# wangty537/raft_optical_flow

Hardware: AMD Instinct MI355X
Metric: image-pairs/s at Sintel 436x1024, 32 iters; corr-lookup GB/s vs HBM peak (higher is better)
Workload: dtype fp32 (convs: f16x3 split MFMA, fp32 accumulate); 1 GPU; RAFT-full inference, 436x1024 padded to 440x1024, 1 pair(s)/GPU/step, iters=32, all-pairs corr, hipGraph; global_batch=1, parallelism=frame-pair sharding x1

## Files before the change

raft_optical_flow_amd/csrc/lookup_conv.hip:

```cpp
#include "lookup_common.hpp"

namespace raft {
namespace {

constexpr int LC_TH = 2, LC_TW = 16, LC_M = 32;
constexpr int LC_R = 4, LC_L = 4, LC_RD = 9;
constexpr int LC_NTAP = LC_L * LC_RD * LC_RD;
constexpr int LC_KS = (LC_NTAP + 31) / 32;
constexpr int LC_N = 256;
constexpr int LC_F1N = 128;
constexpr int LC_F1K = 7, LC_F1KK = 49;
constexpr int LC_F1KS = (2 * LC_F1KK + 31) / 32;
constexpr int LC_FPH = LC_TH + LC_F1K - 1, LC_FPW = LC_TW + LC_F1K - 1;
constexpr int LC_PX = 4;

constexpr int LC_A_BYTES = LC_KS * LC_M * 128;
constexpr int LC_A1_BYTES = LC_F1KS * LC_M * 128;
constexpr int LC_FL_BYTES = LC_FPH * LC_FPW * 8;
constexpr int LC_PATCH_FLOATS = 16 * patch_rs<4>();
constexpr int LC_PATCH_BYTES = 8 * 2 * LC_PATCH_FLOATS * 4;
constexpr int LC_YT_BYTES = 8 * LC_PX * LC_L * LC_RD * 16;
constexpr int LC_OFF_A1 = LC_A_BYTES, LC_OFF_FL = LC_OFF_A1 + LC_A1_BYTES, LC_OFF_PATCH = LC_OFF_FL + LC_FL_BYTES,
              LC_OFF_YT = LC_OFF_PATCH + LC_PATCH_BYTES, LC_LDS = LC_OFF_YT + LC_YT_BYTES;
static_assert(LC_LDS <= 160 * 1024, "LDS budget");

struct LookupConvArgs {
  LookupArgs a;
  const h8* wfrag;
  const float* bias;
  float* out;
  int out_ld;
  int* out_flag;
  const h8* f1frag;
  const float* f1bias;
  float* f1out;
  int f1out_ld;
  int* f1flag;
  int tx_n, ty_n;
  int span_slot;
};

constexpr int LC_SPAN_SLOTS = 256;
__device__ unsigned long long g_lc_span[2 * LC_SPAN_SLOTS];
int g_lc_span_next = -1;

__device__ __forceinline__ void wave_sync() {
  __builtin_amdgcn_fence(__ATOMIC_RELEASE, "wavefront");
  __builtin_amdgcn_wave_barrier();
  __builtin_amdgcn_fence(__ATOMIC_ACQUIRE, "wavefront");
}

template <bool X3, bool BF>
__device__ __forceinline__ void split1(float x, _Float16& hi, _Float16& lo) {
  if constexpr (BF) {
    hi = __builtin_bit_cast(_Float16, (__bf16)x);
  } else {
    hi = (_Float16)x;
    if constexpr (X3) lo = (_Float16)(x - (float)hi);
  }
}

#ifdef LC_STAMPS
__device__ unsigned long long g_lcstamp[16 * 16384];
__device__ __forceinline__ unsigned long long lc_clock() {
  unsigned long long t;
  __builtin_amdgcn_sched_barrier(0);
  asm volatile("s_memtime %0\n\ts_waitcnt lgkmcnt(0)" : "=s"(t)::"memory");
  __builtin_amdgcn_sched_barrier(0);
  return t;
}
__device__ __forceinline__ unsigned long long lc_real() {
  unsigned long long t;
  __builtin_amdgcn_sched_barrier(0);
  asm volatile("s_memrealtime %0\n\ts_waitcnt lgkmcnt(0)" : "=s"(t)::"memory");
  __builtin_amdgcn_sched_barrier(0);
  return t;
}
#define LC_STAMP(k) lc_t[k] = lc_clock()
#else
#define LC_STAMP(k)
#endif

template <int PREC>
__global__ __launch_bounds__(512) void lookup_conv_kernel(LookupConvArgs g) {
#ifdef LC_STAMPS
  unsigned long long lc_t[10];
  const unsigned long long lc_r0 = lc_real();
  LC_STAMP(0);
#endif
  constexpr bool X3 = PREC == RAFT_PREC_F16X3;
  constexpr bool BF = PREC == RAFT_PREC_BF16;
  constexpr int NT = X3 ? 4 : 2;
  constexpr int R = LC_R, RD = LC_RD, WD = 2 * R + 2, RS = patch_rs<4>();
  __shared__ __attribute__((aligned(1024))) char smem[LC_LDS];
  const LookupArgs& a = g.a;
  const int lane = threadIdx.x & 63;
  const int wv = __builtin_amdgcn_readfirstlane(threadIdx.x >> 6);
  const int tile = xcd_tile(blockIdx.x, gridDim.x);
  if (g.span_slot >= 0 && threadIdx.x == 0)
    atomicMin(&g_lc_span[2 * g.span_slot], (unsigned long long)__builtin_amdgcn_s_memrealtime());
  const int per = g.tx_n * g.ty_n;
  const int b = tile / per, sr = tile - b * per;
  const int y0 = (sr / g.tx_n) * LC_TH, x0 = (sr % g.tx_n) * LC_TW;
  const int H = a.H, W = a.W, P = H * W;

#ifndef LC_PF
#define LC_PF 3
#endif
#ifndef LC_TAPS2
#define LC_TAPS2 1
#endif
#ifndef LC_A1EARLY
#define LC_A1EARLY 0
#endif
  constexpr int PF = LC_PF;
  h8 wb[PF + 1][NT];
  auto load_w = [&](int j, h8 (&dst)[NT]) {
    const h8* wf = j < LC_KS ? g.wfrag + ((j * (LC_N / 32) + wv) * 4) * 64
                             : g.f1frag + (((j - LC_KS) * (LC_F1N / 32) + wv) * 4) * 64;
#pragma unroll
    for (int t = 0; t < NT; ++t) dst[t] = wf[t * 64 + lane];
  };

  const int ti = lane >> 4, tj = (lane >> 2) & 3, rr = lane & 3;
  const int lrow = ti * 4 + rr;
  int lth[LC_L], ltw[LC_L];
  unsigned lmsz[LC_L];
  const float* lbs[LC_L];
#pragma unroll
  for (int l = 0; l < LC_L; ++l) {
    lth[l] = a.lv[l].th;
    ltw[l] = a.lv[l].tw;
    lmsz[l] = (unsigned)a.lv[l].mapsz;
    lbs[l] = a.lbase[l];
  }
  float px_x[LC_PX], px_y[LC_PX];
  int px_gp[LC_PX];
  bool px_ok[LC_PX];
#pragma unroll
  for (int k = 0; k < LC_PX; ++k) {
    const int mk = LC_PX * wv + k;
    const int yy = y0 + (mk >> 4), xx = x0 + (mk & 15);
    const bool ok = yy < H && xx < W;
    px_ok[k] = ok;
    px_gp[k] = ok ? b * P + yy * W + xx : b * P;
  }
  {
    int gk = px_gp[0];
#pragma unroll
    for (int k = 1; k < LC_PX; ++k) gk = (lane & 3) == k ? px_gp[k] : gk;
    const float cx = a.coords[2L * gk], cy = a.coords[2L * gk + 1];
#ifdef LC_EARLY
    __builtin_amdgcn_sched_barrier(0);
#pragma unroll
    for (int j = 0; j < PF; ++j) load_w(j, wb[j]);
    __builtin_amdgcn_sched_barrier(0);
#endif
#pragma unroll
    for (int k = 0; k < LC_PX; ++k) {
      px_x[k] = __int_as_float(__builtin_amdgcn_readlane(__float_as_int(cx), k));
      px_y[k] = __int_as_float(__builtin_amdgcn_readlane(__float_as_int(cy), k));
    }
  }
#ifdef LC_STAMPS
  asm volatile("" ::"v"(px_x[0]), "v"(px_y[LC_PX - 1]));
  LC_STAMP(7);
#endif
  const bool col = lane < LC_L * RD;
  int lq = 0;
#pragma unroll
  for (int k = 1; k < LC_L; ++k) lq += lane >= k * RD ? 1 : 0;
  const int l = col ? lq : 0;
  const int ix = lane - l * RD;
  const f32x4 prm = a.prm[l];
  const int fi = threadIdx.x;
  const int fyy = y0 - 3 + fi / LC_FPW, fxx = x0 - 3 + fi % LC_FPW;
  const bool fin = fi < LC_FPH * LC_FPW && (unsigned)fyy < (unsigned)H && (unsigned)fxx < (unsigned)W;
  f32x2 fc = {0.f, 0.f};
  if (fin) fc = *reinterpret_cast<const f32x2*>(a.coords + 2L * ((long)b * P + fyy * W + fxx));
  const int m = lane & 31, h = lane >> 5;
  const float c1b = g.bias ? g.bias[32 * wv + m] : 0.f;
  const float f1b = (wv < 4 && g.f1bias) ? g.f1bias[32 * wv + m] : 0.f;
#ifndef LC_EARLYWAIT
#define LC_EARLYWAIT 1
#endif
  if constexpr (LC_EARLYWAIT != 0) asm volatile("" ::"v"(prm), "v"(c1b), "v"(f1b), "v"(fc));

  __builtin_amdgcn_sched_barrier(0);
  f32x4 v[LC_PX][LC_L];
#ifndef LC_OFF32
#define LC_OFF32 1
#endif
#ifndef LC_TAB
#define LC_TAB 1
#endif
  bool off32 = LC_OFF32 != 0;
  const unsigned nmaps = (unsigned)(a.B * P);
#pragma unroll
  for (int l = 0; l < LC_L; ++l) off32 &= (unsigned long long)nmaps * lmsz[l] * 4ull < 0x7FFFFFF0ull;
  if (off32) {
    __amdgpu_buffer_rsrc_t rsl[LC_L];
    unsigned lano[LC_L], lmsz4[LC_L];
#pragma unroll
    for (int l = 0; l < LC_L; ++l) {
      rsl[l] = __builtin_amdgcn_make_buffer_rsrc(const_cast<float*>(lbs[l]), (short)0, (int)(nmaps * lmsz[l] * 4u),
                                                 0x00020000);
      lano[l] = __umul24((unsigned)ti, (unsigned)(64 * ltw[l])) + 16u * (unsigned)(lane & 15);
      lmsz4[l] = lmsz[l] * 4u;
    }
#if LC_TAB
    int t_sb, t_row, t_col;
    {
      const int ik = (lane >> 2) & 3, il = lane & 3;
      float fx = px_x[0], fy = px_y[0];
      int gpk = px_gp[0];
      bool okk = px_ok[0];
#pragma unroll
      for (int k = 1; k < LC_PX; ++k) {
        fx = ik == k ? px_x[k] : fx;
        fy = ik == k ? px_y[k] : fy;
        gpk = ik == k ? px_gp[k] : gpk;
        okk = ik == k ? px_ok[k] : okk;
      }
      int thl = lth[0], twl = ltw[0];
      unsigned msl = lmsz4[0];
#pragma unroll
      for (int l = 1; l < LC_L; ++l) {
        thl = il == l ? lth[l] : thl;
        twl = il == l ? ltw[l] : twl;
        msl = il == l ? lmsz4[l] : msl;
      }
      const int wx0 = (floor_origin(fx) >> il) - R, wy0 = (floor_origin(fy) >> il) - R;
      const int tyo = wy0 >> 2, txo = wx0 >> 2;
      const int ntx = ((wx0 + WD - 1) >> 2) - txo + 1;
      const int rlo = max(wy0, 0), rhi = min(wy0 + WD, 4 * thl);
      const int clo = max(txo, 0), chi = min(txo + ntx, twl);
      const int rn = okk ? max(rhi - rlo, 0) : 0, cn = max(chi - clo, 0);
      t_sb = (int)((unsigned)gpk * msl + (unsigned)(tyo * twl + txo) * 64u);
      t_row = ((rlo - 4 * tyo) & 0xFFFF) | (rn << 16);
      t_col = ((clo - txo) & 0xFFFF) | (cn << 16);
    }
#pragma unroll
    for (int k = 0; k < LC_PX; ++k) {
#pragma unroll
      for (int l = 0; l < LC_L; ++l) {
        const unsigned sb = (unsigned)__builtin_amdgcn_readlane(t_sb, 4 * k + l);
        const int rp = __builtin_amdgcn_readlane(t_row, 4 * k + l), cp = __builtin_amdgcn_readlane(t_col, 4 * k + l);
        const bool tok = ((unsigned)(lrow - (rp & 0xFFFF)) < (unsigned)(rp >> 16)) &
                         ((unsigned)(tj - (cp & 0xFFFF)) < (unsigned)(cp >> 16));
        unsigned offv = sb + lano[l];
        asm volatile("" : "+v"(offv));
        const unsigned off = tok ? offv : 0x80000000u;
        v[k][l] = __builtin_bit_cast(f32x4, __builtin_amdgcn_raw_buffer_load_b128(rsl[l], off, 0, 0));
      }
    }
#else
#pragma unroll
    for (int k = 0; k < LC_PX; ++k) {
      const unsigned gp = (unsigned)px_gp[k];
      const int xf = __builtin_amdgcn_readfirstlane(floor_origin(px_x[k]));
      const int yf = __builtin_amdgcn_readfirstlane(floor_origin(px_y[k]));
#pragma unroll
      for (int l = 0; l < LC_L; ++l) {
        const int wx0 = (xf >> l) - R, wy0 = (yf >> l) - R;
        const int tyo = wy0 >> 2, txo = wx0 >> 2;
        const int ntx = ((wx0 + WD - 1) >> 2) - txo + 1;
        const int rowm = 4 * tyo + lrow, colt = txo + tj;
        const bool tok = px_ok[k] & ((unsigned)(rowm - wy0) < (unsigned)WD) & ((unsigned)rowm < (unsigned)(4 * lth[l])) &
                         ((unsigned)tj < (unsigned)ntx) & ((unsigned)colt < (unsigned)ltw[l]);
        const unsigned sb = gp * lmsz4[l] + (unsigned)(tyo * ltw[l] + txo) * 64u;
        unsigned offv = sb + lano[l];
        asm volatile("" : "+v"(offv));
        const unsigned off = tok ? offv : 0x80000000u;
        v[k][l] = __builtin_bit_cast(f32x4, __builtin_amdgcn_raw_buffer_load_b128(rsl[l], off, 0, 0));
      }
    }
#endif
  } else {
#if LC_TAB
    int t_lo, t_hi, t_row, t_col;
    {
      const int ik = (lane >> 2) & 3, il = lane & 3;
      float fx = px_x[0], fy = px_y[0];
      int gpk = px_gp[0];
      bool okk = px_ok[0];
#pragma unroll
      for (int k = 1; k < LC_PX; ++k) {
        fx = ik == k ? px_x[k] : fx;
        fy = ik == k ? px_y[k] : fy;
        gpk = ik == k ? px_gp[k] : gpk;
        okk = ik == k ? px_ok[k] : okk;
      }
      int thl = lth[0], twl = ltw[0];
      unsigned msl = lmsz[0];
      const float* bsl = lbs[0];
#pragma unroll
      for (int l = 1; l < LC_L; ++l) {
        thl = il == l ? lth[l] : thl;
        twl = il == l ? ltw[l] : twl;
        msl = il == l ? lmsz[l] : msl;
        bsl = il == l ? lbs[l] : bsl;
      }
      const int wx0 = (floor_origin(fx) >> il) - R, wy0 = (floor_origin(fy) >> il) - R;
      const int tyo = wy0 >> 2, txo = wx0 >> 2;
      const int ntx = ((wx0 + WD - 1) >> 2) - txo + 1;
      const int rlo = max(wy0, 0), rhi = min(wy0 + WD, 4 * thl);
      const int clo = max(txo, 0), chi = min(txo + ntx, twl);
      const int rn = okk ? max(rhi - rlo, 0) : 0, cn = max(chi - clo, 0);
      const float* wbase = bsl + (long)((unsigned long long)(unsigned)gpk * msl) + ((long)tyo * twl + txo) * 16;
      const unsigned long long wa = reinterpret_cast<unsigned long long>(wbase);
      t_lo = (int)(unsigned)wa;
      t_hi = (int)(unsigned)(wa >> 32);
      t_row = ((rlo - 4 * tyo) & 0xFFFF) | (rn << 16);
      t_col = ((clo - txo) & 0xFFFF) | (cn << 16);
    }
#pragma unroll
    for (int k = 0; k < LC_PX; ++k) {
#pragma unroll
      for (int l = 0; l < LC_L; ++l) {
        const unsigned lo = (unsigned)__builtin_amdgcn_readlane(t_lo, 4 * k + l);
        const unsigned hi = (unsigned)__builtin_amdgcn_readlane(t_hi, 4 * k + l);
        const int rp = __builtin_amdgcn_readlane(t_row, 4 * k + l), cp = __builtin_amdgcn_readlane(t_col, 4 * k + l);
        const bool tok = ((unsigned)(lrow - (rp & 0xFFFF)) < (unsigned)(rp >> 16)) &
                         ((unsigned)(tj - (cp & 0xFFFF)) < (unsigned)(cp >> 16));
        const float* wbase = reinterpret_cast<const float*>(((unsigned long long)hi << 32) | lo);
        const __amdgpu_buffer_rsrc_t rs =
            __builtin_amdgcn_make_buffer_rsrc(const_cast<float*>(wbase), (short)0, 0x7FFFFFFF, 0x00020000);
        unsigned offv = __umul24((unsigned)ti, (unsigned)(64 * ltw[l])) + 16u * (unsigned)(lane & 15);
        asm volatile("" : "+v"(offv));
        const unsigned off = tok ? offv : 0x80000000u;
        v[k][l] = __builtin_bit_cast(f32x4, __builtin_amdgcn_raw_buffer_load_b128(rs, off, 0, 0));
      }
    }
#else
#pragma unroll
  for (int k = 0; k < LC_PX; ++k) {
    const bool ok = px_ok[k];
    const int gp = px_gp[k];
    const int xf = __builtin_amdgcn_readfirstlane(floor_origin(px_x[k]));
    const int yf = __builtin_amdgcn_readfirstlane(floor_origin(px_y[k]));
#pragma unroll
    for (int l = 0; l < LC_L; ++l) {
      const int wx0 = (xf >> l) - R, wy0 = (yf >> l) - R;
      const int tyo = wy0 >> 2, txo = wx0 >> 2;
      const int ntx = ((wx0 + WD - 1) >> 2) - txo + 1;
      const int rlo = max(wy0, 0), rhi = min(wy0 + WD, 4 * lth[l]);
      const int clo = max(txo, 0), chi = min(txo + ntx, ltw[l]);
      const int rb = __builtin_amdgcn_readfirstlane(rlo - 4 * tyo), cb = __builtin_amdgcn_readfirstlane(clo - txo);
      const bool tok = ok && ((unsigned)(lrow - rb) < (unsigned)max(rhi - rlo, 0)) &&
                       ((unsigned)(tj - cb) < (unsigned)max(chi - clo, 0));
      const float* wbase = lbs[l] + (long)((unsigned long long)(unsigned)gp * lmsz[l]) + ((long)tyo * ltw[l] + txo) * 16;
      const __amdgpu_buffer_rsrc_t rs =
          __builtin_amdgcn_make_buffer_rsrc(const_cast<float*>(wbase), (short)0, 0x7FFFFFFF, 0x00020000);
      const unsigned off = tok ? __umul24((unsigned)ti, (unsigned)(64 * ltw[l])) + 16u * (unsigned)(lane & 15)
                               : 0x80000000u;
      v[k][l] = __builtin_bit_cast(f32x4, __builtin_amdgcn_raw_buffer_load_b128(rs, off, 0, 0));
    }
  }
#endif
  }
  LC_STAMP(1);
  int4* ytab = reinterpret_cast<int4*>(smem + LC_OFF_YT) + wv * LC_PX * LC_L * RD;
  int xw[LC_PX], xi[LC_PX];
  float xt[LC_PX];
  bool onp[LC_PX];
#pragma unroll
  for (int k = 0; k < LC_PX; ++k) {
    const float s = __builtin_ldexpf(1.0f, -l);
    const int xf = __builtin_amdgcn_readfirstlane(floor_origin(px_x[k]));
    const int yf = __builtin_amdgcn_readfirstlane(floor_origin(px_y[k]));
    axis_entry<R>(px_x[k] * s, xf >> l, ix, prm[0], prm[1], xw[k], xt[k], xi[k]);
    int yw, yi;
    float yt;
    axis_entry<R, true>(px_y[k] * s, yf >> l, ix, prm[2], prm[3], yw, yt, yi);
    onp[k] = xw[k] >= 0 && yw >= 0;
    if (col) ytab[k * LC_L * RD + lane] = int4{yw >= 0 ? yw * RS * 4 : yw, __float_as_int(yt), __float_as_int(1.0f - yt), yi};
  }
  float2* fl = reinterpret_cast<float2*>(smem + LC_OFF_FL);
  if (fi < LC_FPH * LC_FPW) {
    float2 fv = {0.f, 0.f};
    if (fin) {
      fv.x = fc[0] - (float)fxx;
      fv.y = fc[1] - (float)fyy;
    }
    fl[fi] = fv;
  }
  LC_STAMP(2);
#if LC_A1EARLY
  __syncthreads();
  {
    const int mm = threadIdx.x >> 4, q = threadIdx.x & 15;
    const int py = mm >> 4, px = mm & 15;
    float e[8];
#pragma unroll
    for (int i = 0; i < 8; ++i) {
      const int k = 8 * q + i, t = k >> 1;
      const int dy = t / LC_F1K, dx = t - dy * LC_F1K;
      const float2 fv = fl[(py + (k < 2 * LC_F1KK ? dy : 0)) * LC_FPW + px + (k < 2 * LC_F1KK ? dx : 0)];
      e[i] = k < 2 * LC_F1KK ? ((k & 1) ? fv.y : fv.x) : 0.f;
    }
    h8 hi, lo;
    split8<X3, BF>(f32x4{e[0], e[1], e[2], e[3]}, f32x4{e[4], e[5], e[6], e[7]}, hi, lo);
    const int j = q >> 2, qd = q & 3, sw = (mm >> 1) & 7;
    char* row = smem + LC_OFF_A1 + j * (LC_M * 128) + mm * 128;
    *reinterpret_cast<h8*>(row + ((qd ^ sw) << 4)) = hi;
    if constexpr (X3) *reinterpret_cast<h8*>(row + (((4 + qd) ^ sw) << 4)) = lo;
  }
#endif

#ifndef LC_EARLY
#pragma unroll
  for (int j = 0; j < PF; ++j) load_w(j, wb[j]);
#endif
  char* Abase = smem;
  bool big = false;
  auto patch_of = [&](int k) {
    return reinterpret_cast<float*>(smem + LC_OFF_PATCH) + (wv * 2 + (k & 1)) * LC_PATCH_FLOATS;
  };
  const int cbase = l * RD * RD + ix * RD;
  auto taps = [&](int k, float (&val)[RD]) {
    const float* patch = patch_of(k);
    const int4* yt = ytab + k * LC_L * RD;
    const float ex = 1.0f - xt[k];
    const int xwk = xw[k];
    if (__all(!col || onp[k])) {
      if (col) {
        const char* p0 = reinterpret_cast<const char*>(&patch[pidx<4>(0, xwk, l)]);
        const char* p1 = reinterpret_cast<const char*>(&patch[pidx<4>(0, xwk + 1, l)]);
        auto at = [](const char* bp, int byte) { return *reinterpret_cast<const float*>(bp + byte); };
#ifndef LC_TAPS3
#define LC_TAPS3 1
#endif
#if LC_TAPS3 && LC_TAPS2
        int ro[RD];
        float tyv[RD];
        bool cons = true;
#pragma unroll
        for (int iy = 0; iy < RD; ++iy) {
          const int2 ye = *reinterpret_cast<const int2*>(&yt[l * RD + iy]);
          ro[iy] = ye.x;
          tyv[iy] = __int_as_float(ye.y);
        }
#pragma unroll
        for (int iy = 1; iy < RD; ++iy) cons &= ro[iy] == ro[0] + iy * (4 * RS);
        if (__all(cons)) {
          const char* q0 = p0 + ro[0];
          const char* q1 = p1 + ro[0];
          float a0[RD + 1], a1[RD + 1];
#pragma unroll
          for (int r = 0; r <= RD; ++r) {
            a0[r] = at(q0, r * (4 * RS));
            a1[r] = at(q1, r * (4 * RS));
          }
#pragma unroll
          for (int iy = 0; iy < RD; ++iy) {
            const float ty = tyv[iy], sS = 1.0f - ty;
            const f32x2 c0 = {a0[iy], a0[iy + 1]}, c1 = {a1[iy], a1[iy + 1]};
            const f32x2 hh = __builtin_elementwise_fma(c0, (f32x2){ex, ex}, c1 * (f32x2){xt[k], xt[k]});
            val[iy] = fmaf(sS, hh.x, ty * hh.y);
          }
        } else {
#pragma unroll
          for (int iy = 0; iy < RD; ++iy) {
            const float ty = tyv[iy], sS = 1.0f - ty;
            const f32x2 c0 = {at(p0, ro[iy]), at(p0, ro[iy] + 4 * RS)}, c1 = {at(p1, ro[iy]), at(p1, ro[iy] + 4 * RS)};
            const f32x2 hh = __builtin_elementwise_fma(c0, (f32x2){ex, ex}, c1 * (f32x2){xt[k], xt[k]});
            val[iy] = fmaf(sS, hh.x, ty * hh.y);
          }
        }
#else
#pragma unroll
        for (int iy = 0; iy < RD; ++iy) {
#if LC_TAPS2
          const int2 ye = *reinterpret_cast<const int2*>(&yt[l * RD + iy]);
          const int ro = ye.x;
          const float ty = __int_as_float(ye.y), sS = 1.0f - ty;
#else
          const int4 ye = yt[l * RD + iy];
          const int ro = ye.x;
          const float ty = __int_as_float(ye.y), sS = __int_as_float(ye.z);
#endif
          const f32x2 c0 = {at(p0, ro), at(p0, ro + 4 * RS)}, c1 = {at(p1, ro), at(p1, ro + 4 * RS)};
          const f32x2 hh = __builtin_elementwise_fma(c0, (f32x2){ex, ex}, c1 * (f32x2){xt[k], xt[k]});
          val[iy] = fmaf(sS, hh.x, ty * hh.y);
        }
#ifndef LC_TAPSGB
#define LC_TAPSGB 1
#endif
#if LC_TAPSGB && LC_TAPS2
        __builtin_amdgcn_sched_group_barrier(0x100, RD, 0);
        __builtin_amdgcn_sched_group_barrier(0x100, 2 * RD, 0);
        __builtin_amdgcn_sched_group_barrier(0x002, 4 * RD, 0);
#endif
#endif
      }
    } else if (col) {
      unsigned deferred = 0;
#pragma unroll
      for (int iy = 0; iy < RD; ++iy) {
        const int4 ye = yt[l * RD + iy];
        const int yw2 = ye.x;
        const float ty = __int_as_float(ye.y), sS = __int_as_float(ye.z);
        const bool on = (xwk | yw2) >= 0;
        const bool nan = xwk == NAN_POS || yw2 == NAN_POS;
        const int r0 = on ? yw2 / (4 * RS) : 0, c0 = on ? xwk : 0;
        const float vv = patch[pidx<4>(r0, c0, l)] * (sS * ex) + patch[pidx<4>(r0, c0 + 1, l)] * (sS * xt[k]) +
                         patch[pidx<4>(r0 + 1, c0, l)] * (ty * ex) + patch[pidx<4>(r0 + 1, c0 + 1, l)] * (ty * xt[k]);
        val[iy] = nan ? __builtin_nanf("") : vv;
        deferred |= (!on && !nan) ? 1u << iy : 0u;
      }
      if (deferred != 0) {
        const Level& lvl = a.lv[l];
        const float* mp = a.pyr + lvl.off + (long)px_gp[k] * lvl.mapsz;
        auto at = [&](int yy, int xx) {
          return ((unsigned)yy < (unsigned)lvl.h && (unsigned)xx < (unsigned)lvl.w) ? mp[tiled_index(yy, xx, lvl.tw)]
                                                                                    : 0.f;
        };
#pragma unroll
        for (int iy = 0; iy < RD; ++iy) {
          if (!((deferred >> iy) & 1u)) continue;
          const int4 ye = yt[l * RD + iy];
          const int yi = ye.w;
          const float ty = __int_as_float(ye.y), sS = __int_as_float(ye.z);
          val[iy] = at(yi, xi[k]) * (sS * ex) + at(yi, xi[k] + 1) * (sS * xt[k]) + at(yi + 1, xi[k]) * (ty * ex) +
                    at(yi + 1, xi[k] + 1) * (ty * xt[k]);
        }
      }
    }
  };
  auto write_row = [&](int k, const float (&val)[RD]) {
    const int mk = LC_PX * wv + k;
    const int sw = (mk >> 1) & 7;
#if LC_TAPS2
    if (col) {
      const int par = cbase & 1;
      float vv[RD];
#pragma unroll
      for (int iy = 0; iy < RD; ++iy) {
        vv[iy] = px_ok[k] ? val[iy] : 0.f;
        big |= fabsf(vv[iy]) > RAFT_RANGE_LIMIT;
      }
      auto at_c = [&](int c, int half) {
        const int j = c >> 5, kk = c & 31;
        return Abase + j * (LC_M * 128) + mk * 128 + (((4 * half + (kk >> 3)) ^ sw) << 4) + 2 * (kk & 7);
      };
#pragma unroll
      for (int q = 0; q < 4; ++q) {
        const float a0 = par ? vv[2 * q + 1] : vv[2 * q], a1 = par ? vv[2 * q + 2] : vv[2 * q + 1];
        _Float16 h0, l0, h1, l1;
        split1<X3, BF>(a0, h0, l0);
        split1<X3, BF>(a1, h1, l1);
        const int c = cbase + 2 * q + par;
        *reinterpret_cast<h2*>(at_c(c, 0)) = h2{h0, h1};
        if constexpr (X3) *reinterpret_cast<h2*>(at_c(c, 1)) = h2{l0, l1};
      }
      {
        const float a = par ? vv[0] : vv[RD - 1];
        _Float16 hs, ls;
        split1<X3, BF>(a, hs, ls);
        const int c = cbase + (par ? 0 : RD - 1);
        *reinterpret_cast<_Float16*>(at_c(c, 0)) = hs;
        if constexpr (X3) *reinterpret_cast<_Float16*>(at_c(c, 1)) = ls;
      }
    } else if (lane - LC_L * RD < 32 * LC_KS - LC_NTAP) {
#else
    if (col) {
#pragma unroll
      for (int iy = 0; iy < RD; ++iy) {
        const float vv = px_ok[k] ? val[iy] : 0.f;
        big |= fabsf(vv) > RAFT_RANGE_LIMIT;
        const int c = cbase + iy;
        const int j = c >> 5, kk = c & 31;
        _Float16 hi, lo;
        split1<X3, BF>(vv, hi, lo);
        char* rb = Abase + j * (LC_M * 128) + mk * 128;
        *reinterpret_cast<_Float16*>(rb + (((kk >> 3) ^ sw) << 4) + 2 * (kk & 7)) = hi;
        if constexpr (X3) *reinterpret_cast<_Float16*>(rb + (((4 + (kk >> 3)) ^ sw) << 4) + 2 * (kk & 7)) = lo;
      }
    } else if (lane - LC_L * RD < 32 * LC_KS - LC_NTAP) {
#endif
      const int c = LC_NTAP + lane - LC_L * RD;
      const int j = c >> 5, kk = c & 31;
      char* rb = Abase + j * (LC_M * 128) + mk * 128;
      *reinterpret_cast<_Float16*>(rb + (((kk >> 3) ^ sw) << 4) + 2 * (kk & 7)) = (_Float16)0.f;
      if constexpr (X3) *reinterpret_cast<_Float16*>(rb + (((4 + (kk >> 3)) ^ sw) << 4) + 2 * (kk & 7)) = (_Float16)0.f;
    }
    if (a.flow && lane < 2 && px_ok[k]) {
      const int p = px_gp[k] - b * P;
      const float gcoord = lane == 0 ? (float)(p % W) : (float)(p / W);
      a.flow[(long)px_gp[k] * a.flow_ld + lane] = (lane == 0 ? px_x[k] : px_y[k]) - gcoord;
    }
  };
#pragma unroll
  for (int k = 0; k < LC_PX; k += 2) {
#pragma unroll
    for (int lv_ = 0; lv_ < LC_L; ++lv_) {
      *reinterpret_cast<f32x4*>(&patch_of(k)[pidx<4>(lrow, tj * 4, lv_)]) = v[k][lv_];
      *reinterpret_cast<f32x4*>(&patch_of(k + 1)[pidx<4>(lrow, tj * 4, lv_)]) = v[k + 1][lv_];
    }
    wave_sync();
    float va[RD], vb[RD];
    taps(k, va);
    taps(k + 1, vb);
    write_row(k, va);
    write_row(k + 1, vb);
    wave_sync();
  }
  if (a.range_flag && big) *a.range_flag = 1;
  LC_STAMP(3);
#if LC_A1EARLY
  __syncthreads();
#else
  __syncthreads();
  {
    const int mm = threadIdx.x >> 4, q = threadIdx.x & 15;
    const int py = mm >> 4, px = mm & 15;
    float e[8];
#pragma unroll
    for (int i = 0; i < 8; ++i) {
      const int k = 8 * q + i, t = k >> 1;
      const int dy = t / LC_F1K, dx = t - dy * LC_F1K;
      const float2 fv = fl[(py + (k < 2 * LC_F1KK ? dy : 0)) * LC_FPW + px + (k < 2 * LC_F1KK ? dx : 0)];
      e[i] = k < 2 * LC_F1KK ? ((k & 1) ? fv.y : fv.x) : 0.f;
    }
    h8 hi, lo;
    split8<X3, BF>(f32x4{e[0], e[1], e[2], e[3]}, f32x4{e[4], e[5], e[6], e[7]}, hi, lo);
    const int j = q >> 2, qd = q & 3, sw = (mm >> 1) & 7;
    char* row = smem + LC_OFF_A1 + j * (LC_M * 128) + mm * 128;
    *reinterpret_cast<h8*>(row + ((qd ^ sw) << 4)) = hi;
    if constexpr (X3) *reinterpret_cast<h8*>(row + (((4 + qd) ^ sw) << 4)) = lo;
  }
  __syncthreads();
#endif
  LC_STAMP(4);

  const int sw = (m >> 1) & 7;
  auto kstep = [&](const char* A, const h8 (&B)[NT], f32x16& c, f32x16& cx) {
    const char* row = A + m * 128;
    h8 ah[2], al[2];
#pragma unroll
    for (int qq = 0; qq < 2; ++qq) {
      ah[qq] = *reinterpret_cast<const h8*>(row + (((2 * h + qq) ^ sw) << 4));
      if constexpr (X3) al[qq] = *reinterpret_cast<const h8*>(row + (((4 + 2 * h + qq) ^ sw) << 4));
    }
#pragma unroll
    for (int qq = 0; qq < 2; ++qq) {
      if constexpr (BF) {
        c = __builtin_amdgcn_mfma_f32_32x32x16_bf16(__builtin_bit_cast(bf8, ah[qq]), __builtin_bit_cast(bf8, B[qq]), c,
                                                    0, 0, 0);
      } else {
        c = __builtin_amdgcn_mfma_f32_32x32x16_f16(ah[qq], B[qq], c, 0, 0, 0);
      }
      if constexpr (X3) {
        cx = __builtin_amdgcn_mfma_f32_32x32x16_f16(ah[qq], B[2 + qq], cx, 0, 0, 0);
        c = __builtin_amdgcn_mfma_f32_32x32x16_f16(al[qq], B[qq], c, 0, 0, 0);
      }
    }
  };
  f32x16 acc = {}, accx = {}, facc = {}, faccx = {};
  const bool f1w = wv < LC_F1N / 32;
#ifndef LC_SGB
#define LC_SGB 1
#endif
  if constexpr (LC_SGB) {
    struct AF {
      h8 ah[2], al[2];
    };
    auto read_af = [&](const char* A, AF& f) {
      const char* row = A + m * 128;
#pragma unroll
      for (int qq = 0; qq < 2; ++qq) {
        f.ah[qq] = *reinterpret_cast<const h8*>(row + (((2 * h + qq) ^ sw) << 4));
        if constexpr (X3) f.al[qq] = *reinterpret_cast<const h8*>(row + (((4 + 2 * h + qq) ^ sw) << 4));
      }
    };
    auto mfma_af = [&](const AF& f, const h8 (&B)[NT], f32x16& c, f32x16& cx) {
#pragma unroll
      for (int qq = 0; qq < 2; ++qq) {
        if constexpr (BF) {
          c = __builtin_amdgcn_mfma_f32_32x32x16_bf16(__builtin_bit_cast(bf8, f.ah[qq]), __builtin_bit_cast(bf8, B[qq]),
                                                      c, 0, 0, 0);
        } else {
          c = __builtin_amdgcn_mfma_f32_32x32x16_f16(f.ah[qq], B[qq], c, 0, 0, 0);
        }
        if constexpr (X3) {
          cx = __builtin_amdgcn_mfma_f32_32x32x16_f16(f.ah[qq], B[2 + qq], cx, 0, 0, 0);
          c = __builtin_amdgcn_mfma_f32_32x32x16_f16(f.al[qq], B[qq], c, 0, 0, 0);
        }
      }
    };
    auto load_w_any = [&](int j, h8 (&dst)[NT]) {
      const int wq = j < LC_KS ? wv : (wv < LC_F1N / 32 ? wv : LC_F1N / 32 - 1);
      const h8* wf = j < LC_KS ? g.wfrag + ((j * (LC_N / 32) + wq) * 4) * 64
                               : g.f1frag + (((j - LC_KS) * (LC_F1N / 32) + wq) * 4) * 64;
#pragma unroll
      for (int t = 0; t < NT; ++t) dst[t] = wf[t * 64 + lane];
    };
    constexpr int NRA = X3 ? 4 : 2, NMA = X3 ? 6 : 2;
    auto groups = [&](bool loads) {
      if (loads) __builtin_amdgcn_sched_group_barrier(0x020, NT, 0);
#pragma unroll
      for (int i = 0; i < NMA; ++i) {
        if (i < NRA) __builtin_amdgcn_sched_group_barrier(0x100, 1, 0);
        __builtin_amdgcn_sched_group_barrier(0x008, 1, 0);
      }
    };
    AF af[2];
    read_af(Abase, af[0]);
#pragma unroll
    for (int j = 0; j < LC_KS; ++j) {
      __builtin_amdgcn_sched_barrier(0);
      if (j + PF < LC_KS + LC_F1KS) load_w_any(j + PF, wb[(j + PF) % (PF + 1)]);
      read_af(j + 1 < LC_KS ? Abase + (j + 1) * (LC_M * 128) : smem + LC_OFF_A1, af[(j + 1) & 1]);
      mfma_af(af[j & 1], wb[j % (PF + 1)], acc, accx);
      groups(j + PF < LC_KS + LC_F1KS);
      __builtin_amdgcn_sched_barrier(0);
    }
    if (f1w) {
#pragma unroll
      for (int j = LC_KS; j < LC_KS + LC_F1KS; ++j) {
        __builtin_amdgcn_sched_barrier(0);
        if (j + PF < LC_KS + LC_F1KS) load_w_any(j + PF, wb[(j + PF) % (PF + 1)]);
        if (j + 1 < LC_KS + LC_F1KS) read_af(smem + LC_OFF_A1 + (j + 1 - LC_KS) * (LC_M * 128), af[(j + 1) & 1]);
        mfma_af(af[j & 1], wb[j % (PF + 1)], facc, faccx);
        __builtin_amdgcn_sched_barrier(0);
      }
    }
  } else {
#pragma unroll
  for (int j = 0; j < LC_KS; ++j) {
    if (j + PF < LC_KS || f1w) load_w(j + PF, wb[(j + PF) % (PF + 1)]);
    kstep(Abase + j * (LC_M * 128), wb[j % (PF + 1)], acc, accx);
  }
  if (f1w) {
#pragma unroll
    for (int j = LC_KS; j < LC_KS + LC_F1KS; ++j) {
      if (j + PF < LC_KS + LC_F1KS) load_w(j + PF, wb[(j + PF) % (PF + 1)]);
      kstep(smem + LC_OFF_A1 + (j - LC_KS) * (LC_M * 128), wb[j % (PF + 1)], facc, faccx);
    }
  }
  }
  if constexpr (X3) {
#pragma unroll
    for (int r = 0; r < 16; ++r) {
      acc[r] += accx[r] * (1.0f / SPLIT_SCALE);
      facc[r] += faccx[r] * (1.0f / SPLIT_SCALE);
    }
  }
#ifdef LC_STAMPS
  asm volatile("" ::"v"(acc[0]), "v"(acc[15]), "v"(facc[0]));
#endif
  LC_STAMP(5);

  auto store = [&](const f32x16& c, float bias, float* out, int ld, int n, int* flag) {
    bool obig = false;
#pragma unroll
    for (int r = 0; r < 16; ++r) {
      const int mm = (r & 3) + 8 * (r >> 2) + 4 * h;
      const int yy = y0 + (mm >> 4), xx = x0 + (mm & 15);
      const float o = fmaxf(c[r] + bias, 0.f);
      if (yy < H && xx < W) {
        obig |= o > RAFT_RANGE_LIMIT;
        out[((long)b * P + yy * W + xx) * ld + n] = o;
      }
    }
    if (flag && obig) *flag = 1;
  };
  store(acc, c1b, g.out, g.out_ld, 32 * wv + m, g.out_flag);
  if (wv < LC_F1N / 32) store(facc, f1b, g.f1out, g.f1out_ld, 32 * wv + m, g.f1flag);
  if (g.span_slot >= 0) {
    __builtin_amdgcn_s_waitcnt(0);
    __syncthreads();
    if (threadIdx.x == 0)
      atomicMax(&g_lc_span[2 * g.span_slot + 1], (unsigned long long)__builtin_amdgcn_s_memrealtime());
  }
#ifdef LC_END_FENCE
  __builtin_amdgcn_fence(__ATOMIC_RELEASE, "agent");
  __builtin_amdgcn_s_waitcnt(0);
#endif
#ifdef LC_STAMPS
  __builtin_amdgcn_s_waitcnt(0);
  LC_STAMP(6);
  const unsigned long long lc_r1 = lc_real();
  const unsigned wid = blockIdx.x * 8 + wv;
  if (lane == 0 && wid < 16384) {
    unsigned long long* gs = g_lcstamp + wid * 16;
    gs[0] = lc_r0;
    gs[1] = lc_r1;
    for (int k = 0; k < 7; ++k) gs[2 + k] = lc_t[k];
    gs[9] = lc_t[7];
  }
#endif
}

__global__ void lookup_conv_pack_kernel(const h8* __restrict__ split, int k_steps, int nsub, h8* __restrict__ out) {
  const int i = blockIdx.x * blockDim.x + threadIdx.x;
  const int total = k_steps * nsub * 4 * 64;
  if (i >= total) return;
  const int lane = i & 63, t = (i >> 6) & 3, rest = i >> 8;
  const int s = rest % nsub, j = rest / nsub;
  const int n = 32 * s + (lane & 31), hh = lane >> 5, qq = t & 1, lo = t >> 1;
  out[i] = split[((long)n * k_steps + j) * 8 + lo * 4 + 2 * hh + qq];
}

}
}

using namespace raft;

#ifdef LC_STAMPS
extern "C" int raft_debug_lcstamps(unsigned long long* host, int n) {
  return (int)hipMemcpyFromSymbol(host, HIP_SYMBOL(g_lcstamp), sizeof(unsigned long long) * (size_t)n);
}
#endif

extern "C" size_t raft_lookup_conv_weight_floats(int n, int k_pad) {
  if (n <= 0 || n % 32 || k_pad <= 0) return 0;
  return (size_t)((k_pad + 31) / 32) * (size_t)n * 32;
}

extern "C" int raft_lookup_conv_pack_weight(const void* split_weight, int n_pad, int k_pad, int n, void* out,
                                            raft_stream_t stream) {
  RAFT_REQUIRE(split_weight && out && n > 0 && n % 32 == 0 && n <= n_pad && k_pad > 0 && k_pad % 32 == 0,
               "raft_lookup_conv_pack_weight: bad arguments");
  RAFT_REQUIRE((((uintptr_t)split_weight | (uintptr_t)out) & 15) == 0, "raft_lookup_conv_pack_weight: 16-B alignment");
  const int ks = k_pad / 32, nsub = n / 32;
  const int total = ks * nsub * 256;
  hipLaunchKernelGGL(lookup_conv_pack_kernel, dim3((unsigned)cdiv(total, 256)), dim3(256), 0, as_stream(stream),
                     reinterpret_cast<const h8*>(split_weight), ks, nsub, reinterpret_cast<h8*>(out));
  return check_launch("raft_lookup_conv_pack_weight");
}

extern "C" int raft_corr_lookup_conv(const float* pyramid, int B, int H, int W, int L, int radius, const float* coords,
                                     float* flow_out, int flow_ld, int* range_flag, int precision,
                                     const void* c1_weight, const float* c1_bias, int c1_n, float* c1_out,
                                     int c1_out_ld, int* c1_range_flag, const void* f1_weight, const float* f1_bias,
                                     int f1_n, int f1_k, float* f1_out, int f1_out_ld, int* f1_range_flag,
                                     raft_stream_t stream) {
  RAFT_REQUIRE(L == LC_L && radius == LC_R, "raft_corr_lookup_conv: radius 4 and 4 levels only (got %d, %d)", radius,
               L);
  RAFT_REQUIRE(c1_n == LC_N && f1_n == LC_F1N && f1_k == LC_F1K,
               "raft_corr_lookup_conv: convc1 256 / convf1 128 outputs, convf1 7x7 only");
  RAFT_REQUIRE(precision == RAFT_PREC_F16X3 || precision == RAFT_PREC_F16 || precision == RAFT_PREC_BF16,
               "raft_corr_lookup_conv: precision must be F16X3, F16 or BF16 (got %d)", precision);
  RAFT_REQUIRE(c1_weight && c1_out && c1_out_ld >= c1_n && f1_weight && f1_out && f1_out_ld >= f1_n,
               "raft_corr_lookup_conv: bad conv arguments");
  RAFT_REQUIRE((((uintptr_t)c1_weight | (uintptr_t)f1_weight) & 15) == 0 && ((uintptr_t)coords & 7) == 0,
               "raft_corr_lookup_conv: 16-B aligned weights, 8-B aligned coords");
  LookupConvArgs g;
  int rc = lookup_args(g.a, pyramid, B, H, W, L, radius, coords, 0, c1_out, LC_NTAP, 0, flow_out, flow_ld, range_flag);
  if (rc) return rc;
  g.wfrag = reinterpret_cast<const h8*>(c1_weight);
  g.bias = c1_bias;
  g.out = c1_out;
  g.out_ld = c1_out_ld;
  g.out_flag = c1_range_flag;
  g.f1frag = reinterpret_cast<const h8*>(f1_weight);
  g.f1bias = f1_bias;
  g.f1out = f1_out;
  g.f1out_ld = f1_out_ld;
  g.f1flag = f1_range_flag;
  g.tx_n = cdiv(W, LC_TW);
  g.ty_n = cdiv(H, LC_TH);
  hipStreamCaptureStatus cap = hipStreamCaptureStatusNone;
  const bool capturing = hipStreamIsCapturing(as_stream(stream), &cap) == hipSuccess && cap != hipStreamCaptureStatusNone;
  g.span_slot = !capturing && g_lc_span_next >= 0 && g_lc_span_next < LC_SPAN_SLOTS ? g_lc_span_next++ : -1;
  const long nt = (long)B * g.tx_n * g.ty_n;
  RAFT_REQUIRE(nt < (1L << 31), "raft_corr_lookup_conv: grid too large");
  hipStream_t s = as_stream(stream);
  const dim3 grid((unsigned)nt);
  if (precision == RAFT_PREC_F16X3)
    hipLaunchKernelGGL(lookup_conv_kernel<RAFT_PREC_F16X3>, grid, dim3(512), 0, s, g);
  else if (precision == RAFT_PREC_F16)
    hipLaunchKernelGGL(lookup_conv_kernel<RAFT_PREC_F16>, grid, dim3(512), 0, s, g);
  else
    hipLaunchKernelGGL(lookup_conv_kernel<RAFT_PREC_BF16>, grid, dim3(512), 0, s, g);
  return check_launch("raft_corr_lookup_conv");
}

extern "C" int raft_debug_launch_span(int enable) {
  using namespace raft;
  unsigned long long init[2 * LC_SPAN_SLOTS];
  for (int i = 0; i < LC_SPAN_SLOTS; ++i) {
    init[2 * i] = ~0ull;
    init[2 * i + 1] = 0ull;
  }
  const hipError_t e = hipMemcpyToSymbol(HIP_SYMBOL(g_lc_span), init, sizeof(init));
  if (e != hipSuccess) return set_error((int)e, "raft_debug_launch_span: %s", hipGetErrorString(e));
  g_lc_span_next = enable ? 0 : -1;
  return 0;
}
extern "C" int raft_debug_launch_span_read(unsigned long long* host, int n) {
  using namespace raft;
  RAFT_REQUIRE(host && n > 0 && n <= 2 * LC_SPAN_SLOTS, "raft_debug_launch_span_read: bad arguments");
  const hipError_t e = hipMemcpyFromSymbol(host, HIP_SYMBOL(g_lc_span), sizeof(unsigned long long) * (size_t)n);
  if (e != hipSuccess) return set_error((int)e, "raft_debug_launch_span_read: %s", hipGetErrorString(e));
  return 0;
}
```

Before: 139.6 image-pairs/s.

## Redistribute correlation-lookup bilinear taps across all 64 lanes with LDS x-table

Adds a taps64 path that splits the 324 lookup taps per pixel into 108 three-row tasks spread over all 64 lanes (two slots each), instead of having only the 36 column lanes compute nine taps each. A new LDS x-table holds the packed patch column offsets and x weights so any lane can fetch them. Results are written as paired fp16 hi/lo values straight into the swizzled A-fragment layout. The old path remains as a fallback when any pixel falls off the patch, at the cost of extra LDS, more index setup and more code.

```diff
diff --git a/raft_optical_flow_amd/csrc/lookup_conv.hip b/raft_optical_flow_amd/csrc/lookup_conv.hip
--- a/raft_optical_flow_amd/csrc/lookup_conv.hip
+++ b/raft_optical_flow_amd/csrc/lookup_conv.hip
@@ -20,8 +20,10 @@
 constexpr int LC_PATCH_FLOATS = 16 * patch_rs<4>();
 constexpr int LC_PATCH_BYTES = 8 * 2 * LC_PATCH_FLOATS * 4;
 constexpr int LC_YT_BYTES = 8 * LC_PX * LC_L * LC_RD * 16;
+constexpr int LC_XT_BYTES = 8 * LC_PX * LC_L * LC_RD * 8;
 constexpr int LC_OFF_A1 = LC_A_BYTES, LC_OFF_FL = LC_OFF_A1 + LC_A1_BYTES, LC_OFF_PATCH = LC_OFF_FL + LC_FL_BYTES,
-              LC_OFF_YT = LC_OFF_PATCH + LC_PATCH_BYTES, LC_LDS = LC_OFF_YT + LC_YT_BYTES;
+              LC_OFF_YT = LC_OFF_PATCH + LC_PATCH_BYTES, LC_OFF_XT = LC_OFF_YT + LC_YT_BYTES,
+              LC_LDS = LC_OFF_XT + LC_XT_BYTES;
 static_assert(LC_LDS <= 160 * 1024, "LDS budget");
 
 struct LookupConvArgs {
@@ -110,6 +112,13 @@
 #ifndef LC_TAPS2
 #define LC_TAPS2 1
 #endif
+#ifndef LC_TAPS3
+#define LC_TAPS3 1
+#endif
+#ifndef LC_TAPS64
+#define LC_TAPS64 1
+#endif
+#define LC_T64 (LC_TAPS64 && LC_TAPS3 && LC_TAPS2)
 #ifndef LC_A1EARLY
 #define LC_A1EARLY 0
 #endif
@@ -361,6 +370,9 @@
   }
   LC_STAMP(1);
   int4* ytab = reinterpret_cast<int4*>(smem + LC_OFF_YT) + wv * LC_PX * LC_L * RD;
+#if LC_T64
+  int2* xtab = reinterpret_cast<int2*>(smem + LC_OFF_XT) + wv * LC_PX * LC_L * RD;
+#endif
   int xw[LC_PX], xi[LC_PX];
   float xt[LC_PX];
   bool onp[LC_PX];
@@ -375,6 +387,12 @@
     axis_entry<R, true>(px_y[k] * s, yf >> l, ix, prm[2], prm[3], yw, yt, yi);
     onp[k] = xw[k] >= 0 && yw >= 0;
     if (col) ytab[k * LC_L * RD + lane] = int4{yw >= 0 ? yw * RS * 4 : yw, __float_as_int(yt), __float_as_int(1.0f - yt), yi};
+#if LC_T64
+    if (col)
+      xtab[k * LC_L * RD + lane] =
+          int2{(int)((unsigned)(4 * pidx<4>(0, xw[k], l)) | ((unsigned)(4 * pidx<4>(0, xw[k] + 1, l)) << 16)),
+               __float_as_int(xt[k])};
+#endif
   }
   float2* fl = reinterpret_cast<float2*>(smem + LC_OFF_FL);
   if (fi < LC_FPH * LC_FPW) {
@@ -428,9 +446,6 @@
         const char* p0 = reinterpret_cast<const char*>(&patch[pidx<4>(0, xwk, l)]);
         const char* p1 = reinterpret_cast<const char*>(&patch[pidx<4>(0, xwk + 1, l)]);
         auto at = [](const char* bp, int byte) { return *reinterpret_cast<const float*>(bp + byte); };
-#ifndef LC_TAPS3
-#define LC_TAPS3 1
-#endif
 #if LC_TAPS3 && LC_TAPS2
         int ro[RD];
         float tyv[RD];
@@ -591,6 +606,122 @@
       a.flow[(long)px_gp[k] * a.flow_ld + lane] = (lane == 0 ? px_x[k] : px_y[k]) - gcoord;
     }
   };
+#if LC_T64
+  constexpr int NP = 2, NTASK = LC_L * RD * 3;
+  int t_xo[NP], t_yo[NP];
+  int t_pa[NP], t_pq[NP];
+  int t_sa[NP], t_sq[NP];
+  bool t_par[NP];
+#pragma unroll
+  for (int s = 0; s < NP; ++s) {
+    const int ur = lane + 64 * s;
+    const int u = ur < NTASK ? ur : NTASK - 1;
+    const int cu = u / 3, rg = u - 3 * cu;
+    t_xo[s] = cu * 8;
+    t_yo[s] = ((cu / RD) * RD + 3 * rg) * 16;
+    const int c3 = 3 * u, par = c3 & 1;
+    t_par[s] = par != 0;
+    const int cp = ur < NTASK ? c3 + par : LC_NTAP + 2 * (ur - NTASK), cs = par ? c3 : c3 + 2;
+    auto off_c = [&](int c) { return (c >> 5) * (LC_M * 128) + LC_PX * wv * 128 + 2 * (c & 7); };
+    t_pa[s] = off_c(cp < 32 * LC_KS ? cp : 0);
+    t_pq[s] = ((cp & 31) >> 3) << 4;
+    t_sa[s] = off_c(cs);
+    t_sq[s] = ((cs & 31) >> 3) << 4;
+  }
+  auto taps64 = [&](int k, float (&val)[NP][3]) {
+    const char* patch = reinterpret_cast<const char*>(patch_of(k));
+    const char* ytb = reinterpret_cast<const char*>(ytab + k * LC_L * RD);
+    const char* xtb = reinterpret_cast<const char*>(xtab + k * LC_L * RD);
+    auto at = [](const char* bp, int byte) { return *reinterpret_cast<const float*>(bp + byte); };
+    int ro[NP][3];
+    float tyv[NP][3], xtv[NP];
+    const char *p0[NP], *p1[NP];
+    bool cons = true;
+#pragma unroll
+    for (int s = 0; s < NP; ++s) {
+      const int2 xe = *reinterpret_cast<const int2*>(xtb + t_xo[s]);
+      p0[s] = patch + (xe.x & 0xFFFF);
+      p1[s] = patch + ((unsigned)xe.x >> 16);
+      xtv[s] = __int_as_float(xe.y);
+#pragma unroll
+      for (int i = 0; i < 3; ++i) {
+        const int2 ye = *reinterpret_cast<const int2*>(ytb + t_yo[s] + 16 * i);
+        ro[s][i] = ye.x;
+        tyv[s][i] = __int_as_float(ye.y);
+      }
+      cons &= (ro[s][1] == ro[s][0] + 4 * RS) & (ro[s][2] == ro[s][0] + 8 * RS);
+    }
+    if (__all(cons)) {
+#pragma unroll
+      for (int s = 0; s < NP; ++s) {
+        const char* q0 = p0[s] + ro[s][0];
+        const char* q1 = p1[s] + ro[s][0];
+        const float ex = 1.0f - xtv[s];
+        float a0[4], a1[4];
+#pragma unroll
+        for (int r = 0; r < 4; ++r) {
+          a0[r] = at(q0, r * (4 * RS));
+          a1[r] = at(q1, r * (4 * RS));
+        }
+#pragma unroll
+        for (int i = 0; i < 3; ++i) {
+          const float ty = tyv[s][i], sS = 1.0f - ty;
+          const f32x2 c0 = {a0[i], a0[i + 1]}, c1 = {a1[i], a1[i + 1]};
+          const f32x2 hh = __builtin_elementwise_fma(c0, (f32x2){ex, ex}, c1 * (f32x2){xtv[s], xtv[s]});
+          val[s][i] = fmaf(sS, hh.x, ty * hh.y);
+        }
+      }
+    } else {
+#pragma unroll
+      for (int s = 0; s < NP; ++s) {
+        const float ex = 1.0f - xtv[s];
+#pragma unroll
+        for (int i = 0; i < 3; ++i) {
+          const float ty = tyv[s][i], sS = 1.0f - ty;
+          const int r = ro[s][i];
+          const f32x2 c0 = {at(p0[s], r), at(p0[s], r + 4 * RS)}, c1 = {at(p1[s], r), at(p1[s], r + 4 * RS)};
+          const f32x2 hh = __builtin_elementwise_fma(c0, (f32x2){ex, ex}, c1 * (f32x2){xtv[s], xtv[s]});
+          val[s][i] = fmaf(sS, hh.x, ty * hh.y);
+        }
+      }
+    }
+  };
+  auto write64 = [&](int k, const float (&val)[NP][3]) {
+    const int mk = LC_PX * wv + k;
+    const int sw4 = ((mk >> 1) & 7) << 4;
+#pragma unroll
+    for (int s = 0; s < NP; ++s) {
+      const bool task = s == 0 || lane < NTASK - 64;
+      const bool pad = s == 1 && lane < NTASK - 64 + (32 * LC_KS - LC_NTAP) / 2;
+      float vv[3];
+#pragma unroll
+      for (int i = 0; i < 3; ++i) {
+        vv[i] = (px_ok[k] && task) ? val[s][i] : 0.f;
+        big |= fabsf(vv[i]) > RAFT_RANGE_LIMIT;
+      }
+      const float a0 = t_par[s] ? vv[1] : vv[0], a1 = t_par[s] ? vv[2] : vv[1], as = t_par[s] ? vv[0] : vv[2];
+      _Float16 h0, l0, h1, l1, hs, ls;
+      split1<X3, BF>(a0, h0, l0);
+      split1<X3, BF>(a1, h1, l1);
+      split1<X3, BF>(as, hs, ls);
+      char* pp = Abase + k * 128 + t_pa[s];
+      char* ps = Abase + k * 128 + t_sa[s];
+      if (task || pad) {
+        *reinterpret_cast<h2*>(pp + (t_pq[s] ^ sw4)) = h2{h0, h1};
+        if constexpr (X3) *reinterpret_cast<h2*>(pp + (t_pq[s] ^ sw4 ^ 64)) = h2{l0, l1};
+      }
+      if (task) {
+        *reinterpret_cast<_Float16*>(ps + (t_sq[s] ^ sw4)) = hs;
+        if constexpr (X3) *reinterpret_cast<_Float16*>(ps + (t_sq[s] ^ sw4 ^ 64)) = ls;
+      }
+    }
+    if (a.flow && lane < 2 && px_ok[k]) {
+      const int p = px_gp[k] - b * P;
+      const float gcoord = lane == 0 ? (float)(p % W) : (float)(p / W);
+      a.flow[(long)px_gp[k] * a.flow_ld + lane] = (lane == 0 ? px_x[k] : px_y[k]) - gcoord;
+    }
+  };
+#endif
 #pragma unroll
   for (int k = 0; k < LC_PX; k += 2) {
 #pragma unroll
@@ -599,11 +730,22 @@
       *reinterpret_cast<f32x4*>(&patch_of(k + 1)[pidx<4>(lrow, tj * 4, lv_)]) = v[k + 1][lv_];
     }
     wave_sync();
-    float va[RD], vb[RD];
-    taps(k, va);
-    taps(k + 1, vb);
-    write_row(k, va);
-    write_row(k + 1, vb);
+#if LC_T64
+    if (__all(!col || (onp[k] && onp[k + 1]))) {
+      float va[NP][3], vb[NP][3];
+      taps64(k, va);
+      taps64(k + 1, vb);
+      write64(k, va);
+      write64(k + 1, vb);
+    } else
+#endif
+    {
+      float va[RD], vb[RD];
+      taps(k, va);
+      taps(k + 1, vb);
+      write_row(k, va);
+      write_row(k + 1, vb);
+    }
     wave_sync();
   }
   if (a.range_flag && big) *a.range_flag = 1;
```

Result: no change. 140.5 image-pairs/s, median of 6 (+0.6%).
